# pyannote/pyannote-audio

Measured on NVIDIA H100. Metric: audio-hours/sec (RTF) community-1 diarization, 16kHz mono, 1/2/4/8 H100, higher is better.
Workload: dtype f16 tensor-core trunk (f32 accumulate) + split-f16x3 tensor-core segmentation (f32-level accuracy) + f64 clustering

## Files before the change

### pyannote_audio_b200/csrc/api.cu

```cuda
#include "../../include/b200diar.h"
#include "audio.cuh"
#include "cluster.cuh"
#include "common.cuh"
#include "emb.cuh"
#include "post.cuh"
#include "seg.cuh"
#include "ssl.cuh"
#include <algorithm>
#include <climits>
#include <cmath>
#include <cstdlib>

using namespace b200;

constexpr int kXvecLayers = 5;
constexpr int kXvecMinSamples = 4771;
constexpr int kXvecStatsLd = 3008;
struct XvecWeights {
  bool loaded = false;
  SincNetWeights sinc;
  int taps[kXvecLayers] = {5, 3, 3, 1, 1}, dil[kXvecLayers] = {1, 2, 3, 1, 1};
  int cin_pad[kXvecLayers] = {64, 512, 512, 512, 512}, cout_pad[kXvecLayers] = {512, 512, 512, 512, 1536};
  __half* w_hi[kXvecLayers] = {};
  __half* w_lo[kXvecLayers] = {};
// ... 365 lines not shown
        }
    if ((rc = upload_split(ctx, whh_wg, &S.w_hh_hi[l], &S.w_hh_lo[l]))) return rc;
  }
  const int lin_in[2] = {256, 128};
  for (int i = 0; i < 2; ++i) {
    B200_CHECK(w->linear_weight[i] && w->linear_bias[i], B200_ERR_INVALID, "linear.%d missing", i);
    std::vector<float> lw(w->linear_weight[i], w->linear_weight[i] + 128 * lin_in[i]), lb(w->linear_bias[i], w->linear_bias[i] + 128);
    if ((rc = upload_split(ctx, lw, &S.lin_w_hi[i], &S.lin_w_lo[i]))) return rc;
    if ((rc = upload(ctx, lw, &S.lin_w[i]))) return rc;
    if ((rc = upload(ctx, lb, &S.lin_b[i]))) return rc;
  }
  B200_CHECK(w->classifier_weight && w->classifier_bias, B200_ERR_INVALID, "classifier missing");
  std::vector<float> cw(w->classifier_weight, w->classifier_weight + (size_t)num_classes * 128),
      cb(w->classifier_bias, w->classifier_bias + num_classes);
  if ((rc = upload(ctx, cw, &S.cls_w))) return rc;
  if ((rc = upload(ctx, cb, &S.cls_b))) return rc;
  return B200_OK;
}

}

extern "C" {

const char* b200_last_error(void) { return b200::last_error(); }
int b200_version(void) { return 100; }

int b200_ctx_create(b200_ctx** out, int device) {
  B200_CHECK(out != nullptr, B200_ERR_INVALID, "ctx pointer is NULL");
  int ndev = 0;
  B200_CUDA_OK(cudaGetDeviceCount(&ndev));
  B200_CHECK(device >= 0 && device < ndev, B200_ERR_INVALID, "device %d not available (%d devices)", device, ndev);
  cudaDeviceProp prop;
  B200_CUDA_OK(cudaGetDeviceProperties(&prop, device));
  B200_CHECK(prop.major == 9 && prop.minor == 0, B200_ERR_STATE,
             "device %d is sm_%d%d; this library is built for sm_90a (H100) only", device, prop.major, prop.minor);
  b200_ctx* c = new b200_ctx();
  c->device = device;
  c->num_sms = prop.multiProcessorCount;
  if (const char* e = std::getenv("B200_CONV_IMPL")) c->conv_impl = std::atoi(e);
  if (const char* e = std::getenv("B200_EMB_MAX_BATCH")) c->emb_max_batch = std::atoi(e) > 0 ? std::atoi(e) : c->emb_max_batch;
  if (const char* e = std::getenv("B200_SEG_MAX_BATCH")) c->seg_max_batch = std::atoi(e) > 0 ? std::atoi(e) : c->seg_max_batch;
  *out = c;
  return B200_OK;
}

int b200_ctx_destroy(b200_ctx* ctx) {
  if (!ctx) return B200_OK;
  DeviceGuard g(ctx->device);
  cudaDeviceSynchronize();
  for (void* p : ctx->owned_seg) cudaFree(p);
  for (void* p : ctx->owned_emb) cudaFree(p);
  for (void* p : ctx->owned_xvec) cudaFree(p);
  for (void* p : ctx->owned_ssl) cudaFree(p);
  for (auto& t : ctx->resample_tables) cudaFree(t.dev);
  if (ctx->ws) cudaFree(ctx->ws);
  if (ctx->d_off) cudaFree(ctx->d_off);
  if (ctx->d_valid) cudaFree(ctx->d_valid);
  if (ctx->d_frame0) cudaFree(ctx->d_frame0);
  if (ctx->d_runs) cudaFree(ctx->d_runs);
  delete ctx;
  return B200_OK;
}

int b200_ctx_set_option(b200_ctx* ctx, const char* key, int64_t value) {
  B200_CHECK(ctx && key, B200_ERR_INVALID, "NULL ctx/key");
  std::string k(key);
  if (k == "conv_impl") ctx->conv_impl = (int)value;
  else if (k == "seg_max_batch") ctx->seg_max_batch = (int)value;
  else if (k == "emb_max_batch") ctx->emb_max_batch = (int)value;
  else if (k == "ssl_max_batch") ctx->ssl_max_batch = (int)value;
  else if (k == "profile") ctx->profile = (int)value;
  else if (k == "seg_gemm_impl") ctx->seg_gemm_impl = (int)value;
  else if (k == "seg_conv_impl") ctx->seg_conv_impl = (int)value;
  else if (k == "seg_rec_impl") ctx->seg_rec_impl = (int)value;
  else if (k == "fbank_share") ctx->fbank_share = (int)value;
  else if (k == "linkage_grid_min") {
    B200_CHECK(value >= 2 && value <= kLinkGridMinDefault, B200_ERR_INVALID, "option '%s' value %lld out of range",
               key, (long long)value);
    ctx->linkage_grid_min = (int)value;
  }
  else B200_CHECK(false, B200_ERR_INVALID, "unknown option '%s'", key);
  B200_CHECK(ctx->seg_max_batch >= 1 && ctx->emb_max_batch >= 1 && ctx->ssl_max_batch >= 1 && ctx->conv_impl >= 0 && ctx->conv_impl <= 2 &&
                 ctx->seg_gemm_impl >= 0 && ctx->seg_gemm_impl <= 1 && ctx->seg_conv_impl >= 0 && ctx->seg_conv_impl <= 2 &&
                 ctx->seg_rec_impl >= 0 && ctx->seg_rec_impl <= 1,
             B200_ERR_INVALID, "option '%s' value %lld out of range", key, (long long)value);
  return B200_OK;
}

int64_t b200_ctx_launch_count(const b200_ctx* ctx) { return ctx ? ctx->launches : 0; }

int b200_ctx_timer(b200_ctx* ctx, const char* name, double* total_ms, int64_t* units) {
  B200_CHECK(ctx && name && total_ms && units, B200_ERR_INVALID, "bad arguments");
  DeviceGuard g(ctx->device);
  std::string k(name);
  std::vector<std::pair<cudaEvent_t, cudaEvent_t>>* v = nullptr;
  int64_t* u = nullptr;
  if (k == "trunk") { v = &ctx->trunk_events; u = &ctx->trunk_segments; }
  else if (k == "seg") { v = &ctx->seg_events; u = &ctx->seg_chunks; }
  else B200_CHECK(false, B200_ERR_INVALID, "unknown timer '%s'", name);
  B200_CUDA_OK(cudaDeviceSynchronize());
  double ms = 0.0;
  for (auto& pr : *v) {
    float t = 0.f;
    B200_CUDA_OK(cudaEventElapsedTime(&t, pr.first, pr.second));
    ms += t;
    ctx->event_pool.push_back(pr.first);
    ctx->event_pool.push_back(pr.second);
  }
  v->clear();
  *total_ms = ms;
  *units = *u;
  *u = 0;
  return B200_OK;
}

static int64_t gcd64(int64_t a, int64_t b) { while (b) { const int64_t t = a % b; a = b; b = t; } return a; }

int64_t b200_audio_num_frames(int64_t frames_in, int32_t sr_in, int32_t sr_out) {
  if (frames_in <= 0 || sr_in <= 0 || sr_out <= 0) return 0;
  if (sr_in == sr_out) return frames_in;
  const int64_t g = gcd64(sr_in, sr_out), orig = sr_in / g, nw = sr_out / g;
  return (nw * frames_in + orig - 1) / orig;
}

int b200_audio_ingest(b200_ctx* ctx, const void* pcm, int32_t format, int32_t channels, int64_t frames_in,
                      int32_t sr_in, int32_t sr_out, int32_t channel, float* out, int64_t out_capacity, void* stream) {
  B200_CHECK(ctx && pcm && out && channels >= 1 && frames_in >= 0 && sr_in > 0 && sr_out > 0, B200_ERR_INVALID,
             "bad arguments");
  B200_CHECK(format == B200_PCM_S16_INTERLEAVED || format == B200_PCM_F32_PLANAR, B200_ERR_INVALID,
             "unknown PCM format %d", (int)format);
  B200_CHECK(channel < channels, B200_ERR_INVALID, "channel %d of a %d-channel file", (int)channel, (int)channels);
  const int64_t frames_out = b200_audio_num_frames(frames_in, sr_in, sr_out);
  B200_CHECK(frames_out <= out_capacity, B200_ERR_INVALID, "output holds %lld samples, %lld needed",
             (long long)out_capacity, (long long)frames_out);
  if (frames_out == 0) return B200_OK;
  DeviceGuard g(ctx->device);
  const int64_t gg = gcd64(sr_in, sr_out);
  const int orig = (int)(sr_in / gg), nw = (int)(sr_out / gg);
  const b200_ctx::ResampleTable* tab = nullptr;
  for (auto& t : ctx->resample_tables)
    if (t.orig == orig && t.nw == nw) tab = &t;
  if (!tab) {
    b200_ctx::ResampleTable t{orig, nw, 0, nullptr};
    std::vector<float> host;
    if (orig == nw) { host.assign(1, 1.0f); t.width = 0; }
    else resample_table(orig, nw, &t.width, &host);
    B200_CUDA_OK(cudaMalloc((void**)&t.dev, host.size() * sizeof(float)));
    B200_CUDA_OK(cudaMemcpy(t.dev, host.data(), host.size() * sizeof(float), cudaMemcpyHostToDevice));
    ctx->resample_tables.push_back(t);
    tab = &ctx->resample_tables.back();
  }
  ctx->launches += 1;
  return audio_ingest(pcm, format, channels, frames_in, channel, tab->dev, tab->orig, tab->nw, tab->width, out,
                      frames_out, (cudaStream_t)stream);
}

int b200_seg_load_head(b200_ctx* ctx, const b200_seg_weights* w, int32_t num_classes, int32_t activation) {
  B200_CHECK(ctx && w, B200_ERR_INVALID, "NULL ctx/weights");
  B200_CHECK(num_classes >= 1 && num_classes <= kSegMaxClasses, B200_ERR_INVALID,
             "a classifier of %d classes is unsupported (1 .. %d)", (int)num_classes, kSegMaxClasses);
  B200_CHECK(activation == B200_SEG_LOGSOFTMAX || activation == B200_SEG_SIGMOID, B200_ERR_INVALID,
             "unknown classifier activation %d (B200_SEG_LOGSOFTMAX = 0, B200_SEG_SIGMOID = 1)", (int)activation);
  DeviceGuard g(ctx->device);
  SegWeights& S = ctx->seg;
  B200_CHECK(w->lstm_layers >= 1 && w->lstm_layers <= 4, B200_ERR_INVALID, "lstm_layers=%d unsupported",
             (int)w->lstm_layers);
  S.loaded = false;
// ... 1031 lines not shown
```

### pyannote_audio_b200/csrc/seg.cuh

```cuda
#pragma once
#include "common.cuh"

namespace b200 {

constexpr int kSegMinWindow = 1261;
constexpr int kSegTileP = 64;
struct SegGeom {
  int W, sinc_len, pool0, conv1_len, pool1, conv2_len, pool2;
  int tiles0, tiles1, tiles2;
};
inline SegGeom seg_geom(int W) {
  SegGeom g;
  g.W = W;
  g.sinc_len = 1 + (W - kSincK) / kSincStride;
  g.pool0 = g.sinc_len / 3;
  g.conv1_len = g.pool0 - 4;
  g.pool1 = g.conv1_len / 3;
  g.conv2_len = g.pool1 - 4;
  g.pool2 = g.conv2_len / 3;
  g.tiles0 = (g.pool0 + kSegTileP - 1) / kSegTileP;
  g.tiles1 = (g.pool1 + kSegTileP - 1) / kSegTileP;
  g.tiles2 = (g.pool2 + kSegTileP - 1) / kSegTileP;
  return g;
}

struct SincNetWeights {
  float wav_w = 1.f, wav_b = 0.f;
  __half* sinc_wg_hi = nullptr;
  __half* sinc_wg_lo = nullptr;
  float* sinc_f = nullptr;
  float* in_gamma[3] = {nullptr, nullptr, nullptr};
  float* in_beta[3] = {nullptr, nullptr, nullptr};
  float* conv_w[2] = {nullptr, nullptr};
  float* conv_b[2] = {nullptr, nullptr};
  __half* conv_wg_hi[2] = {nullptr, nullptr};
  __half* conv_wg_lo[2] = {nullptr, nullptr};
};

constexpr int kSegLogSoftmax = 0;
constexpr int kSegSigmoid = 1;
constexpr int kSegMaxClasses = 32;

struct SegWeights {
  bool loaded = false;
  int lstm_layers = 4;
  int num_classes = kClasses;
  int activation = kSegLogSoftmax;
  SincNetWeights sinc;
  float* w_ih[8] = {};
  float* b_g[8] = {};
  int k_in[8] = {};
  float* w_hh[8] = {};
  __half* w_hh_hi[8] = {};
  __half* w_hh_lo[8] = {};
  __half* w_ih_hi[8] = {};
  __half* w_ih_lo[8] = {};
  __half* lin_w_hi[2] = {nullptr, nullptr};
  __half* lin_w_lo[2] = {nullptr, nullptr};
  float* lin_w[2] = {nullptr, nullptr};
  float* lin_b[2] = {nullptr, nullptr};
  float* cls_w = nullptr;
  float* cls_b = nullptr;
};

int sgemm_nt(const float* A, int lda, const float* Bw, int ldb, float* C, int ldc, const float* bias, int M, int N,
             int K, int act, cudaStream_t stream);

struct GemmTaps {
  int taps = 1, dil = 0;
  const float* scale = nullptr;
  const float* shift = nullptr;
};
int gemm_tc_split(const __half* A_hi, const __half* A_lo, int lda, const __half* B_hi, const __half* B_lo, int ldb,
                  float* C, int ldc, __half* C_hi, __half* C_lo, int ldc_h, const float* bias, int M, int N, int K,
                  int act, int num_sms, cudaStream_t stream, float* const* C_peers = nullptr, int n_peers = 0,
                  const GemmTaps& taps = GemmTaps());
int split_f16(const float* x, __half* hi, __half* lo, size_t n, cudaStream_t st);
int lstm_rec_wg(const float* Gx, const __half* Wh, const __half* Wl, __half* Yh, __half* Yl, int NB, int T,
                cudaStream_t stream);

int sinc_wg_forward(const SegGeom& g, const float* wav, const long long* chunk_off, const int* chunk_valid,
                    const float2* affine, const __half* Wh, const __half* Wl, int NB, float* P0, double2* part,
                    int impl, cudaStream_t stream);
int conv5_wg_forward(const SegGeom& g, int layer, const float* Pin, const float2* affine, const __half* Wh,
                     const __half* Wl, const float* bias, int NB, float* Pout, double2* part, int impl,
                     cudaStream_t stream);

size_t sincnet_workspace_bytes(const SegGeom& g, int NB);
int sincnet_launches(const SegGeom& g);
int sincnet_forward(const SincNetWeights& W, const SegGeom& g, const float* wav, const long long* chunk_off,
                    const int* chunk_valid, int NB, void* ws, float* x0, int conv_impl, cudaStream_t stream);

struct SegHeadOut {
  unsigned char* cls = nullptr;
  float* logp = nullptr;
  float* scores = nullptr;
  float* max_scores = nullptr;
};
size_t lstm_workspace_bytes(int NB, int T, int k0);
int lstm_head_forward(const SegWeights& W, const float* x0, int NB, int T, void* ws, const SegHeadOut& out,
                      int num_sms, int gemm_impl, int rec_impl, cudaStream_t stream);

}
```

### pyannote_audio_b200/csrc/seg_lstm.cu

```cuda
#include "common.cuh"
#include "seg.cuh"
#include <cooperative_groups.h>
#include <array>
#include <utility>

namespace cg = cooperative_groups;

namespace b200 {

__device__ __forceinline__ float sigmoidf_(float x) { return 1.f / (1.f + expf(-x)); }

template <int RB>
__global__ void __cluster_dims__(2, 1, 1) __launch_bounds__(256, 1)
lstm_rec_kernel(const float* __restrict__ Gx , const float* __restrict__ Whh ,
                float* __restrict__ Y , __half* __restrict__ Yh, __half* __restrict__ Yl,
                int NB, int T, int ntiles) {
  constexpr int NBT = 8 * RB;
  extern __shared__ float sm[];
  float* Ws = sm;
  float* hb = sm + 128 * 256;
  cg::cluster_group cluster = cg::this_cluster();
  const int rank = (int)cluster.block_rank();
  const int cid = blockIdx.x >> 1;
  const int dir = cid / ntiles;
// ... 142 lines not shown
  for (int k = 1; k < K; ++k) mx = fmaxf(mx, v[k]);
  float se = 0.f;
#pragma unroll
  for (int k = 0; k < K; ++k) se += expf(v[k] - mx);
  const float lse = logf(se);
  int best = 0;
  float bv = 0.f;
#pragma unroll
  for (int k = 0; k < K; ++k) {
    const float lp = (v[k] - mx) - lse;
    if (logp) logp[(size_t)row * K + k] = lp;
    if (k == 0 || lp > bv) { bv = lp; best = k; }
  }
  cls[row] = (unsigned char)best;
}

typedef void (*ClassifierFn)(const float*, const float*, const float*, unsigned char*, float*, float*, float*, int);
template <int ACT, int... I>
static std::array<ClassifierFn, sizeof...(I)> classifier_table(std::integer_sequence<int, I...>) {
  return {{&classifier_kernel<I + 1, ACT>...}};
}
static const auto kLogSoftmaxHeads = classifier_table<kSegLogSoftmax>(std::make_integer_sequence<int, kSegMaxClasses>());
static const auto kSigmoidHeads = classifier_table<kSegSigmoid>(std::make_integer_sequence<int, kSegMaxClasses>());

struct LstmWs {
  float *Gx, *Ya, *Yb, *Z1, *Z2;
  __half *Xh, *Xl, *Yah, *Yal, *Ybh, *Ybl, *Z1h, *Z1l;
};
static size_t carve_lstm(int NB, int T, int k0, void* base, LstmWs* w) {
  Workspace ws(base, 256);
  LstmWs t;
  const size_t M = (size_t)NB * T;
  t.Gx = (float*)ws.take(M * 1024 * sizeof(float));
  t.Ya = (float*)ws.take(M * 256 * sizeof(float));
  t.Yb = (float*)ws.take(M * 256 * sizeof(float));
  t.Z1 = (float*)ws.take(M * 128 * sizeof(float));
  t.Z2 = (float*)ws.take(M * 128 * sizeof(float));
  t.Xh = (__half*)ws.take(M * k0 * sizeof(__half));
  t.Xl = (__half*)ws.take(M * k0 * sizeof(__half));
  t.Yah = (__half*)ws.take(M * 256 * sizeof(__half));
  t.Yal = (__half*)ws.take(M * 256 * sizeof(__half));
  t.Ybh = (__half*)ws.take(M * 256 * sizeof(__half));
  t.Ybl = (__half*)ws.take(M * 256 * sizeof(__half));
  t.Z1h = (__half*)ws.take(M * 128 * sizeof(__half));
  t.Z1l = (__half*)ws.take(M * 128 * sizeof(__half));
  if (w) *w = t;
  return ws.bytes();
}
size_t lstm_workspace_bytes(int NB, int T, int k0) { return carve_lstm(NB, T, k0, nullptr, nullptr); }

template <int RB>
static int launch_rec(const float* Gx, const float* Whh, float* Y, __half* Yh, __half* Yl, int NB, int T,
                      cudaStream_t stream) {
  constexpr int NBT = 8 * RB;
  const int ntiles = ceil_div(NB, NBT);
  const size_t smem = (128 * 256 + 2 * 128 * NBT) * sizeof(float);
  B200_CUDA_OK(cudaFuncSetAttribute(lstm_rec_kernel<RB>, cudaFuncAttributeMaxDynamicSharedMemorySize, (int)smem));
  lstm_rec_kernel<RB><<<2 * 2 * ntiles, 256, smem, stream>>>(Gx, Whh, Y, Yh, Yl, NB, T, ntiles);
  B200_CUDA_OK(cudaGetLastError());
  return B200_OK;
}

int lstm_head_forward(const SegWeights& W, const float* x0, int NB, int T, void* ws, const SegHeadOut& out,
                      int num_sms, int gemm_impl, int rec_impl, cudaStream_t stream) {
  LstmWs w;
  carve_lstm(NB, T, W.k_in[0], ws, &w);
  const int M = NB * T;
  const int clusters = num_sms / 2;
  const bool tc = gemm_impl != 0;
  int rc;
  const float* in = x0;
  const __half *in_h = w.Xh, *in_l = w.Xl;
  if (tc && (rc = split_f16(x0, w.Xh, w.Xl, (size_t)M * W.k_in[0], stream))) return rc;
  float* outs[2] = {w.Ya, w.Yb};
  __half* outs_h[2] = {w.Yah, w.Ybh};
  __half* outs_l[2] = {w.Yal, w.Ybl};
  for (int l = 0; l < W.lstm_layers; ++l) {
    if (tc)
      rc = gemm_tc_split(in_h, in_l, W.k_in[l], W.w_ih_hi[l], W.w_ih_lo[l], W.k_in[l], w.Gx, 1024, nullptr, nullptr, 0,
                         W.b_g[l], M, 1024, W.k_in[l], 0, num_sms, stream);
    else
      rc = sgemm_nt(in, W.k_in[l], W.w_ih[l], W.k_in[l], w.Gx, 1024, W.b_g[l], M, 1024, W.k_in[l], 0, stream);
    if (rc) return rc;
    if (tc && rec_impl == 1) {
      if ((rc = lstm_rec_wg(w.Gx, W.w_hh_hi[l], W.w_hh_lo[l], outs_h[l & 1], outs_l[l & 1], NB, T, stream))) return rc;
      in_h = outs_h[l & 1]; in_l = outs_l[l & 1];
      continue;
    }
    float* y = tc ? nullptr : outs[l & 1];
    __half* yh = tc ? outs_h[l & 1] : nullptr;
    __half* yl = tc ? outs_l[l & 1] : nullptr;
    if (2 * ceil_div(NB, 64) >= clusters) rc = launch_rec<8>(w.Gx, W.w_hh[l], y, yh, yl, NB, T, stream);
    else if (2 * ceil_div(NB, 32) >= clusters) rc = launch_rec<4>(w.Gx, W.w_hh[l], y, yh, yl, NB, T, stream);
    else rc = launch_rec<2>(w.Gx, W.w_hh[l], y, yh, yl, NB, T, stream);
    if (rc) return rc;
    in = y; in_h = yh; in_l = yl;
  }
  if (tc) {
    rc = gemm_tc_split(in_h, in_l, 256, W.lin_w_hi[0], W.lin_w_lo[0], 256, nullptr, 0, w.Z1h, w.Z1l, 128, W.lin_b[0], M,
                       128, 256, 1, num_sms, stream);
    if (rc) return rc;
    rc = gemm_tc_split(w.Z1h, w.Z1l, 128, W.lin_w_hi[1], W.lin_w_lo[1], 128, w.Z2, 128, nullptr, nullptr, 0,
                       W.lin_b[1], M, 128, 128, 1, num_sms, stream);
    if (rc) return rc;
  } else {
    rc = sgemm_nt(in, 256, W.lin_w[0], 256, w.Z1, 128, W.lin_b[0], M, 128, 256, 1, stream);
    if (rc) return rc;
    rc = sgemm_nt(w.Z1, 128, W.lin_w[1], 128, w.Z2, 128, W.lin_b[1], M, 128, 128, 1, stream);
    if (rc) return rc;
  }
  const ClassifierFn head = (W.activation == kSegSigmoid ? kSigmoidHeads : kLogSoftmaxHeads)[W.num_classes - 1];
  head<<<ceil_div(M, 8), 256, 0, stream>>>(w.Z2, W.cls_w, W.cls_b, out.cls, out.logp, out.scores, out.max_scores, M);
  B200_CUDA_OK(cudaGetLastError());
  return B200_OK;
}

}
```

### pyannote_audio_b200/csrc/seg_lstm_wg.cu

```cuda
#include "common.cuh"
#include "seg.cuh"
#include "tc_common.cuh"

namespace b200 {

constexpr int kRecThreads = 128;
constexpr int kRecSeqs = 64;
constexpr uint32_t kRecWBox = 256u * 128u;
constexpr uint32_t kRecXOff = 1024u + 4u * kRecWBox;

__device__ __forceinline__ float rec_sigmoid(float x) { return 1.f / (1.f + expf(-x)); }

__device__ __forceinline__ uint32_t pack_h2(float a, float b) {
  __half2 h = __floats2half2_rn(a, b);
  return *reinterpret_cast<uint32_t*>(&h);
}

__global__ void __cluster_dims__(2, 1, 1) __launch_bounds__(kRecThreads, 1)
lstm_rec_wg_kernel(const __grid_constant__ CUtensorMap tmWh, const __grid_constant__ CUtensorMap tmWl,
                   const float* __restrict__ Gx , __half* __restrict__ Yh, __half* __restrict__ Yl,
                   int NB, int T, int ntiles) {
  extern __shared__ uint8_t smem_raw[];
  const uint32_t raw = smem_u32(smem_raw);
  const uint32_t base = (raw + 1023u) & ~1023u;
// ... 33 lines not shown

  float acc[128];
  for (int step = 0; step < T; ++step) {
    const int t = dir ? (T - 1 - step) : step;
#pragma unroll
    for (int i = 0; i < 2; ++i) {
      const bool ok = rows[i] < NB;
      const float4* gp = reinterpret_cast<const float4*>(Gx + ((size_t)(ok ? rows[i] : 0) * T + t) * 1024 + gcol);
#pragma unroll
      for (int jj = 0; jj < 8; ++jj) {
        const float4 u0 = ok ? __ldg(gp + 8 * jj) : make_float4(0.f, 0.f, 0.f, 0.f);
        const float4 u1 = ok ? __ldg(gp + 8 * jj + 1) : make_float4(0.f, 0.f, 0.f, 0.f);
        const float v[8] = {u0.x, u0.y, u0.z, u0.w, u1.x, u1.y, u1.z, u1.w};
#pragma unroll
        for (int g = 0; g < 4; ++g)
#pragma unroll
          for (int e = 0; e < 2; ++e) acc[4 * (4 * jj + g) + 2 * i + e] = v[4 * e + g];
      }
      if (step + 1 < T && ok) {
        const int tn = dir ? t - 1 : t + 1;
        const char* np = reinterpret_cast<const char*>(Gx + ((size_t)rows[i] * T + tn) * 1024 + gcol);
#pragma unroll
        for (int jj = 0; jj < 8; ++jj) asm volatile("prefetch.global.L2 [%0];" ::"l"(np + 128 * jj));
      }
    }
    wg_fence();
#pragma unroll
    for (int ks = 0; ks < 8; ++ks) {
      const int s = ks & 3;
      const uint32_t* xb = xbuf + ((step & 1) * 2 + (ks >> 2)) * 32 * kRecThreads;
      uint32_t ah[4], al[4];
#pragma unroll
      for (int r = 0; r < 4; ++r) {
        const int i = r & 1, jj = 2 * s + (r >> 1);
        ah[r] = xb[(i * 8 + jj) * kRecThreads + tid];
        al[r] = xb[(16 + i * 8 + jj) * kRecThreads + tid];
      }
      const uint32_t wb = w_smem + (uint32_t)(ks >> 2) * kRecWBox + (uint32_t)(ks & 3) * 32u;
      const uint64_t wh = wg_desc(wb, 128), wl = wg_desc(wb + 2 * kRecWBox, 128);
      WgmmaRS<256>::mma(acc, al, wh);
      WgmmaRS<256>::mma(acc, ah, wl);
      WgmmaRS<256>::mma(acc, ah, wh);
    }
    wg_commit();
    wg_wait<0>();
    const uint32_t hoff = (uint32_t)((((step + 1) & 1) * 2 + (int)rank) * 32 * kRecThreads + tid);
    uint32_t* own = xbuf + hoff;
    const uint32_t px = peer_x + hoff * 4u;
#pragma unroll
    for (int i = 0; i < 2; ++i) {
#pragma unroll
      for (int jj = 0; jj < 8; ++jj) {
        float hn[2];
#pragma unroll
        for (int e = 0; e < 2; ++e) {
          const float ig = rec_sigmoid(acc[4 * (4 * jj + 0) + 2 * i + e]);
          const float fg = rec_sigmoid(acc[4 * (4 * jj + 1) + 2 * i + e]);
          const float gg = tanhf(acc[4 * (4 * jj + 2) + 2 * i + e]);
          const float og = rec_sigmoid(acc[4 * (4 * jj + 3) + 2 * i + e]);
          c[i][jj][e] = fmaf(fg, c[i][jj][e], ig * gg);
          hn[e] = og * tanhf(c[i][jj][e]);
        }
        const __half h0 = __float2half_rn(hn[0]), h1 = __float2half_rn(hn[1]);
        const __half2 hi2 = __halves2half2(h0, h1);
        const uint32_t vh = *reinterpret_cast<const uint32_t*>(&hi2);
        const uint32_t vl = pack_h2(hn[0] - __half2float(h0), hn[1] - __half2float(h1));
        own[(i * 8 + jj) * kRecThreads] = vh;
        own[(16 + i * 8 + jj) * kRecThreads] = vl;
        asm volatile("st.shared::cluster.u32 [%0], %1;" ::"r"(px + (uint32_t)((i * 8 + jj) * kRecThreads) * 4u),
                     "r"(vh) : "memory");
        asm volatile("st.shared::cluster.u32 [%0], %1;" ::"r"(px + (uint32_t)((16 + i * 8 + jj) * kRecThreads) * 4u),
                     "r"(vl) : "memory");
        if (rows[i] < NB) {
          const size_t o = ((size_t)rows[i] * T + t) * 256 + dir * 128 + rank * 64 + 8 * jj + 2 * q;
          *reinterpret_cast<uint32_t*>(Yh + o) = vh;
          *reinterpret_cast<uint32_t*>(Yl + o) = vl;
        }
      }
    }
    asm volatile("barrier.cluster.arrive.release.aligned;\n\tbarrier.cluster.wait.acquire.aligned;" ::: "memory");
  }
}

int lstm_rec_wg(const float* Gx, const __half* Wh, const __half* Wl, __half* Yh, __half* Yl, int NB, int T,
                cudaStream_t stream) {
  CUtensorMap tm[2];
  const cuuint64_t dims[3] = {128, 256, 4};
  const cuuint64_t strides[2] = {128 * 2, 256 * 128 * 2};
  const cuuint32_t box[3] = {64, 256, 1};
  int rc;
  for (int h = 0; h < 2; ++h)
    if ((rc = encode_f16_map(&tm[h], 3, h ? Wl : Wh, dims, strides, box, nullptr, CU_TENSOR_MAP_SWIZZLE_128B,
                             "lstm W_hh")))
      return rc;
  const size_t smem = 1024 + kRecXOff + 4u * 32u * kRecThreads * 4u;
  B200_CUDA_OK(cudaFuncSetAttribute(lstm_rec_wg_kernel, cudaFuncAttributeMaxDynamicSharedMemorySize, (int)smem));
  const int ntiles = ceil_div(NB, kRecSeqs);
  lstm_rec_wg_kernel<<<2 * 2 * ntiles, kRecThreads, smem, stream>>>(tm[0], tm[1], Gx, Yh, Yl, NB, T, ntiles);
  B200_CUDA_OK(cudaGetLastError());
  return B200_OK;
}

}
```

### pyannote_audio_b200/csrc/tc_common.cuh

```cuda
#pragma once
#include "common.cuh"
#include <cuda.h>

namespace b200 {

__device__ __forceinline__ uint32_t smem_u32(const void* p) {
  return static_cast<uint32_t>(__cvta_generic_to_shared(p));
}
__device__ __forceinline__ void mbar_init(uint32_t bar, uint32_t count) {
  asm volatile("mbarrier.init.shared::cta.b64 [%0], %1;" ::"r"(bar), "r"(count));
}
__device__ __forceinline__ void mbar_expect_tx(uint32_t bar, uint32_t bytes) {
  asm volatile("mbarrier.arrive.expect_tx.shared::cta.b64 _, [%0], %1;" ::"r"(bar), "r"(bytes) : "memory");
}
__device__ __forceinline__ void mbar_arrive(uint32_t bar) {
  asm volatile("mbarrier.arrive.shared::cta.b64 _, [%0];" ::"r"(bar) : "memory");
}
__device__ __forceinline__ void mbar_arrive_n(uint32_t bar, uint32_t count) {
  asm volatile("mbarrier.arrive.shared::cta.b64 _, [%0], %1;" ::"r"(bar), "r"(count) : "memory");
}
__device__ __forceinline__ void mbar_wait(uint32_t bar, uint32_t parity) {
  asm volatile(
      "{\n\t"
      ".reg .pred p;\n\t"
// ... 52 lines not shown
}
__device__ __forceinline__ void named_bar_sync(int id) { asm volatile("bar.sync %0, 128;" ::"r"(id) : "memory"); }
__device__ __forceinline__ void wg_fence() { asm volatile("wgmma.fence.sync.aligned;" ::: "memory"); }
__device__ __forceinline__ void wg_commit() { asm volatile("wgmma.commit_group.sync.aligned;" ::: "memory"); }
template <int N>
__device__ __forceinline__ void wg_wait() { asm volatile("wgmma.wait_group.sync.aligned %0;" ::"n"(N) : "memory"); }

template <int N>
struct Wgmma;
template <>
struct Wgmma<32> {
  __device__ __forceinline__ static void mma(float* d, uint64_t a, uint64_t b) {
    asm volatile(
        "wgmma.mma_async.sync.aligned.m64n32k16.f32.f16.f16 "
        "{%0, %1, %2, %3, %4, %5, %6, %7, %8, %9, %10, %11, %12, %13, %14, %15}, %16, %17, 1, 1, 1, 0, 0;"
        : "+f"(d[0]), "+f"(d[1]), "+f"(d[2]), "+f"(d[3]), "+f"(d[4]), "+f"(d[5]), "+f"(d[6]), "+f"(d[7]), "+f"(d[8]), "+f"(d[9]), "+f"(d[10]), "+f"(d[11]), "+f"(d[12]), "+f"(d[13]), "+f"(d[14]), "+f"(d[15])
        : "l"(a), "l"(b));
  }
};
template <>
struct Wgmma<64> {
  __device__ __forceinline__ static void mma(float* d, uint64_t a, uint64_t b) {
    asm volatile(
        "wgmma.mma_async.sync.aligned.m64n64k16.f32.f16.f16 "
        "{%0, %1, %2, %3, %4, %5, %6, %7, %8, %9, %10, %11, %12, %13, %14, %15, %16, %17, %18, %19, %20, %21, %22, %23, %24, %25, %26, %27, %28, %29, %30, %31}, %32, %33, 1, 1, 1, 0, 0;"
        : "+f"(d[0]), "+f"(d[1]), "+f"(d[2]), "+f"(d[3]), "+f"(d[4]), "+f"(d[5]), "+f"(d[6]), "+f"(d[7]), "+f"(d[8]), "+f"(d[9]), "+f"(d[10]), "+f"(d[11]), "+f"(d[12]), "+f"(d[13]), "+f"(d[14]), "+f"(d[15]), "+f"(d[16]), "+f"(d[17]), "+f"(d[18]), "+f"(d[19]), "+f"(d[20]), "+f"(d[21]), "+f"(d[22]), "+f"(d[23]), "+f"(d[24]), "+f"(d[25]), "+f"(d[26]), "+f"(d[27]), "+f"(d[28]), "+f"(d[29]), "+f"(d[30]), "+f"(d[31])
        : "l"(a), "l"(b));
  }
};
template <>
struct Wgmma<128> {
  __device__ __forceinline__ static void mma(float* d, uint64_t a, uint64_t b) {
    asm volatile(
        "wgmma.mma_async.sync.aligned.m64n128k16.f32.f16.f16 "
        "{%0, %1, %2, %3, %4, %5, %6, %7, %8, %9, %10, %11, %12, %13, %14, %15, %16, %17, %18, %19, %20, %21, %22, %23, %24, %25, %26, %27, %28, %29, %30, %31, %32, %33, %34, %35, %36, %37, %38, %39, %40, %41, %42, %43, %44, %45, %46, %47, %48, %49, %50, %51, %52, %53, %54, %55, %56, %57, %58, %59, %60, %61, %62, %63}, %64, %65, 1, 1, 1, 0, 0;"
        : "+f"(d[0]), "+f"(d[1]), "+f"(d[2]), "+f"(d[3]), "+f"(d[4]), "+f"(d[5]), "+f"(d[6]), "+f"(d[7]), "+f"(d[8]), "+f"(d[9]), "+f"(d[10]), "+f"(d[11]), "+f"(d[12]), "+f"(d[13]), "+f"(d[14]), "+f"(d[15]), "+f"(d[16]), "+f"(d[17]), "+f"(d[18]), "+f"(d[19]), "+f"(d[20]), "+f"(d[21]), "+f"(d[22]), "+f"(d[23]), "+f"(d[24]), "+f"(d[25]), "+f"(d[26]), "+f"(d[27]), "+f"(d[28]), "+f"(d[29]), "+f"(d[30]), "+f"(d[31]), "+f"(d[32]), "+f"(d[33]), "+f"(d[34]), "+f"(d[35]), "+f"(d[36]), "+f"(d[37]), "+f"(d[38]), "+f"(d[39]), "+f"(d[40]), "+f"(d[41]), "+f"(d[42]), "+f"(d[43]), "+f"(d[44]), "+f"(d[45]), "+f"(d[46]), "+f"(d[47]), "+f"(d[48]), "+f"(d[49]), "+f"(d[50]), "+f"(d[51]), "+f"(d[52]), "+f"(d[53]), "+f"(d[54]), "+f"(d[55]), "+f"(d[56]), "+f"(d[57]), "+f"(d[58]), "+f"(d[59]), "+f"(d[60]), "+f"(d[61]), "+f"(d[62]), "+f"(d[63])
        : "l"(a), "l"(b));
  }
};
template <>
struct Wgmma<256> {
  __device__ __forceinline__ static void mma(float* d, uint64_t a, uint64_t b) {
    asm volatile(
        "wgmma.mma_async.sync.aligned.m64n256k16.f32.f16.f16 "
        "{%0, %1, %2, %3, %4, %5, %6, %7, %8, %9, %10, %11, %12, %13, %14, %15, %16, %17, %18, %19, %20, %21, %22, %23, %24, %25, %26, %27, %28, %29, %30, %31, %32, %33, %34, %35, %36, %37, %38, %39, %40, %41, %42, %43, %44, %45, %46, %47, %48, %49, %50, %51, %52, %53, %54, %55, %56, %57, %58, %59, %60, %61, %62, %63, %64, %65, %66, %67, %68, %69, %70, %71, %72, %73, %74, %75, %76, %77, %78, %79, %80, %81, %82, %83, %84, %85, %86, %87, %88, %89, %90, %91, %92, %93, %94, %95, %96, %97, %98, %99, %100, %101, %102, %103, %104, %105, %106, %107, %108, %109, %110, %111, %112, %113, %114, %115, %116, %117, %118, %119, %120, %121, %122, %123, %124, %125, %126, %127}, %128, %129, 1, 1, 1, 0, 0;"
        : "+f"(d[0]), "+f"(d[1]), "+f"(d[2]), "+f"(d[3]), "+f"(d[4]), "+f"(d[5]), "+f"(d[6]), "+f"(d[7]), "+f"(d[8]), "+f"(d[9]), "+f"(d[10]), "+f"(d[11]), "+f"(d[12]), "+f"(d[13]), "+f"(d[14]), "+f"(d[15]), "+f"(d[16]), "+f"(d[17]), "+f"(d[18]), "+f"(d[19]), "+f"(d[20]), "+f"(d[21]), "+f"(d[22]), "+f"(d[23]), "+f"(d[24]), "+f"(d[25]), "+f"(d[26]), "+f"(d[27]), "+f"(d[28]), "+f"(d[29]), "+f"(d[30]), "+f"(d[31]), "+f"(d[32]), "+f"(d[33]), "+f"(d[34]), "+f"(d[35]), "+f"(d[36]), "+f"(d[37]), "+f"(d[38]), "+f"(d[39]), "+f"(d[40]), "+f"(d[41]), "+f"(d[42]), "+f"(d[43]), "+f"(d[44]), "+f"(d[45]), "+f"(d[46]), "+f"(d[47]), "+f"(d[48]), "+f"(d[49]), "+f"(d[50]), "+f"(d[51]), "+f"(d[52]), "+f"(d[53]), "+f"(d[54]), "+f"(d[55]), "+f"(d[56]), "+f"(d[57]), "+f"(d[58]), "+f"(d[59]), "+f"(d[60]), "+f"(d[61]), "+f"(d[62]), "+f"(d[63]), "+f"(d[64]), "+f"(d[65]), "+f"(d[66]), "+f"(d[67]), "+f"(d[68]), "+f"(d[69]), "+f"(d[70]), "+f"(d[71]), "+f"(d[72]), "+f"(d[73]), "+f"(d[74]), "+f"(d[75]), "+f"(d[76]), "+f"(d[77]), "+f"(d[78]), "+f"(d[79]), "+f"(d[80]), "+f"(d[81]), "+f"(d[82]), "+f"(d[83]), "+f"(d[84]), "+f"(d[85]), "+f"(d[86]), "+f"(d[87]), "+f"(d[88]), "+f"(d[89]), "+f"(d[90]), "+f"(d[91]), "+f"(d[92]), "+f"(d[93]), "+f"(d[94]), "+f"(d[95]), "+f"(d[96]), "+f"(d[97]), "+f"(d[98]), "+f"(d[99]), "+f"(d[100]), "+f"(d[101]), "+f"(d[102]), "+f"(d[103]), "+f"(d[104]), "+f"(d[105]), "+f"(d[106]), "+f"(d[107]), "+f"(d[108]), "+f"(d[109]), "+f"(d[110]), "+f"(d[111]), "+f"(d[112]), "+f"(d[113]), "+f"(d[114]), "+f"(d[115]), "+f"(d[116]), "+f"(d[117]), "+f"(d[118]), "+f"(d[119]), "+f"(d[120]), "+f"(d[121]), "+f"(d[122]), "+f"(d[123]), "+f"(d[124]), "+f"(d[125]), "+f"(d[126]), "+f"(d[127])
        : "l"(a), "l"(b));
  }
};

template <int N>
struct WgmmaRS;
template <>
struct WgmmaRS<32> {
  __device__ __forceinline__ static void mma(float* d, const uint32_t* a, uint64_t b) {
    asm volatile(
        "wgmma.mma_async.sync.aligned.m64n32k16.f32.f16.f16 "
        "{%0, %1, %2, %3, %4, %5, %6, %7, %8, %9, %10, %11, %12, %13, %14, %15}, {%16, %17, %18, %19}, %20, 1, 1, 1, 0;"
        : "+f"(d[0]), "+f"(d[1]), "+f"(d[2]), "+f"(d[3]), "+f"(d[4]), "+f"(d[5]), "+f"(d[6]), "+f"(d[7]), "+f"(d[8]), "+f"(d[9]), "+f"(d[10]), "+f"(d[11]), "+f"(d[12]), "+f"(d[13]), "+f"(d[14]), "+f"(d[15])
        : "r"(a[0]), "r"(a[1]), "r"(a[2]), "r"(a[3]), "l"(b));
  }
};
template <>
struct WgmmaRS<64> {
  __device__ __forceinline__ static void mma(float* d, const uint32_t* a, uint64_t b) {
    asm volatile(
        "wgmma.mma_async.sync.aligned.m64n64k16.f32.f16.f16 "
        "{%0, %1, %2, %3, %4, %5, %6, %7, %8, %9, %10, %11, %12, %13, %14, %15, %16, %17, %18, %19, %20, %21, %22, %23, %24, %25, %26, %27, %28, %29, %30, %31}, {%32, %33, %34, %35}, %36, 1, 1, 1, 0;"
        : "+f"(d[0]), "+f"(d[1]), "+f"(d[2]), "+f"(d[3]), "+f"(d[4]), "+f"(d[5]), "+f"(d[6]), "+f"(d[7]), "+f"(d[8]), "+f"(d[9]), "+f"(d[10]), "+f"(d[11]), "+f"(d[12]), "+f"(d[13]), "+f"(d[14]), "+f"(d[15]), "+f"(d[16]), "+f"(d[17]), "+f"(d[18]), "+f"(d[19]), "+f"(d[20]), "+f"(d[21]), "+f"(d[22]), "+f"(d[23]), "+f"(d[24]), "+f"(d[25]), "+f"(d[26]), "+f"(d[27]), "+f"(d[28]), "+f"(d[29]), "+f"(d[30]), "+f"(d[31])
        : "r"(a[0]), "r"(a[1]), "r"(a[2]), "r"(a[3]), "l"(b));
  }
};
template <>
struct WgmmaRS<80> {
  __device__ __forceinline__ static void mma(float* d, const uint32_t* a, uint64_t b) {
    asm volatile(
        "wgmma.mma_async.sync.aligned.m64n80k16.f32.f16.f16 "
        "{%0, %1, %2, %3, %4, %5, %6, %7, %8, %9, %10, %11, %12, %13, %14, %15, %16, %17, %18, %19, %20, %21, %22, %23, %24, %25, %26, %27, %28, %29, %30, %31, %32, %33, %34, %35, %36, %37, %38, %39}, {%40, %41, %42, %43}, %44, 1, 1, 1, 0;"
        : "+f"(d[0]), "+f"(d[1]), "+f"(d[2]), "+f"(d[3]), "+f"(d[4]), "+f"(d[5]), "+f"(d[6]), "+f"(d[7]), "+f"(d[8]), "+f"(d[9]), "+f"(d[10]), "+f"(d[11]), "+f"(d[12]), "+f"(d[13]), "+f"(d[14]), "+f"(d[15]), "+f"(d[16]), "+f"(d[17]), "+f"(d[18]), "+f"(d[19]), "+f"(d[20]), "+f"(d[21]), "+f"(d[22]), "+f"(d[23]), "+f"(d[24]), "+f"(d[25]), "+f"(d[26]), "+f"(d[27]), "+f"(d[28]), "+f"(d[29]), "+f"(d[30]), "+f"(d[31]), "+f"(d[32]), "+f"(d[33]), "+f"(d[34]), "+f"(d[35]), "+f"(d[36]), "+f"(d[37]), "+f"(d[38]), "+f"(d[39])
        : "r"(a[0]), "r"(a[1]), "r"(a[2]), "r"(a[3]), "l"(b));
  }
};
template <>
struct WgmmaRS<256> {
  __device__ __forceinline__ static void mma(float* d, const uint32_t* a, uint64_t b) {
    asm volatile(
        "wgmma.mma_async.sync.aligned.m64n256k16.f32.f16.f16 "
        "{%0, %1, %2, %3, %4, %5, %6, %7, %8, %9, %10, %11, %12, %13, %14, %15, %16, %17, %18, %19, %20, %21, %22, %23, %24, %25, %26, %27, %28, %29, %30, %31, %32, %33, %34, %35, %36, %37, %38, %39, %40, %41, %42, %43, %44, %45, %46, %47, %48, %49, %50, %51, %52, %53, %54, %55, %56, %57, %58, %59, %60, %61, %62, %63, %64, %65, %66, %67, %68, %69, %70, %71, %72, %73, %74, %75, %76, %77, %78, %79, %80, %81, %82, %83, %84, %85, %86, %87, %88, %89, %90, %91, %92, %93, %94, %95, %96, %97, %98, %99, %100, %101, %102, %103, %104, %105, %106, %107, %108, %109, %110, %111, %112, %113, %114, %115, %116, %117, %118, %119, %120, %121, %122, %123, %124, %125, %126, %127}, {%128, %129, %130, %131}, %132, 1, 1, 1, 0;"
        : "+f"(d[0]), "+f"(d[1]), "+f"(d[2]), "+f"(d[3]), "+f"(d[4]), "+f"(d[5]), "+f"(d[6]), "+f"(d[7]), "+f"(d[8]), "+f"(d[9]), "+f"(d[10]), "+f"(d[11]), "+f"(d[12]), "+f"(d[13]), "+f"(d[14]), "+f"(d[15]), "+f"(d[16]), "+f"(d[17]), "+f"(d[18]), "+f"(d[19]), "+f"(d[20]), "+f"(d[21]), "+f"(d[22]), "+f"(d[23]), "+f"(d[24]), "+f"(d[25]), "+f"(d[26]), "+f"(d[27]), "+f"(d[28]), "+f"(d[29]), "+f"(d[30]), "+f"(d[31]), "+f"(d[32]), "+f"(d[33]), "+f"(d[34]), "+f"(d[35]), "+f"(d[36]), "+f"(d[37]), "+f"(d[38]), "+f"(d[39]), "+f"(d[40]), "+f"(d[41]), "+f"(d[42]), "+f"(d[43]), "+f"(d[44]), "+f"(d[45]), "+f"(d[46]), "+f"(d[47]), "+f"(d[48]), "+f"(d[49]), "+f"(d[50]), "+f"(d[51]), "+f"(d[52]), "+f"(d[53]), "+f"(d[54]), "+f"(d[55]), "+f"(d[56]), "+f"(d[57]), "+f"(d[58]), "+f"(d[59]), "+f"(d[60]), "+f"(d[61]), "+f"(d[62]), "+f"(d[63]), "+f"(d[64]), "+f"(d[65]), "+f"(d[66]), "+f"(d[67]), "+f"(d[68]), "+f"(d[69]), "+f"(d[70]), "+f"(d[71]), "+f"(d[72]), "+f"(d[73]), "+f"(d[74]), "+f"(d[75]), "+f"(d[76]), "+f"(d[77]), "+f"(d[78]), "+f"(d[79]), "+f"(d[80]), "+f"(d[81]), "+f"(d[82]), "+f"(d[83]), "+f"(d[84]), "+f"(d[85]), "+f"(d[86]), "+f"(d[87]), "+f"(d[88]), "+f"(d[89]), "+f"(d[90]), "+f"(d[91]), "+f"(d[92]), "+f"(d[93]), "+f"(d[94]), "+f"(d[95]), "+f"(d[96]), "+f"(d[97]), "+f"(d[98]), "+f"(d[99]), "+f"(d[100]), "+f"(d[101]), "+f"(d[102]), "+f"(d[103]), "+f"(d[104]), "+f"(d[105]), "+f"(d[106]), "+f"(d[107]), "+f"(d[108]), "+f"(d[109]), "+f"(d[110]), "+f"(d[111]), "+f"(d[112]), "+f"(d[113]), "+f"(d[114]), "+f"(d[115]), "+f"(d[116]), "+f"(d[117]), "+f"(d[118]), "+f"(d[119]), "+f"(d[120]), "+f"(d[121]), "+f"(d[122]), "+f"(d[123]), "+f"(d[124]), "+f"(d[125]), "+f"(d[126]), "+f"(d[127])
        : "r"(a[0]), "r"(a[1]), "r"(a[2]), "r"(a[3]), "l"(b));
  }
};

int encode_f16_map(CUtensorMap* tm, int rank, const void* ptr, const cuuint64_t* dims, const cuuint64_t* strides,
                   const cuuint32_t* box, const cuuint32_t* estr, CUtensorMapSwizzle swizzle, const char* what);

}
```

Baseline: 1.908.

## Add two-warpgroup pipelined LSTM recurrence kernel as default rec impl

Adds a new LSTM recurrence kernel that splits the 256 gate columns across two warpgroups, each issuing m64n128 split-f16 wgmma, and prefetches the next step's Gx input while the tensor-core work runs. The cluster barrier is split into arrive and wait halves so the wait for the peer's h exchange overlaps the Yh/Yl global stores. With rec_impl=1 as the default, the new kernel replaces the old one, which stays reachable as impl 2. In exchange the kernel uses more threads and registers and adds a little code complexity.

```diff
diff --git a/pyannote_audio_b200/csrc/api.cu b/pyannote_audio_b200/csrc/api.cu
--- a/pyannote_audio_b200/csrc/api.cu
+++ b/pyannote_audio_b200/csrc/api.cu
@@ -471,7 +471,7 @@
   else B200_CHECK(false, B200_ERR_INVALID, "unknown option '%s'", key);
   B200_CHECK(ctx->seg_max_batch >= 1 && ctx->emb_max_batch >= 1 && ctx->ssl_max_batch >= 1 && ctx->conv_impl >= 0 && ctx->conv_impl <= 2 &&
                  ctx->seg_gemm_impl >= 0 && ctx->seg_gemm_impl <= 1 && ctx->seg_conv_impl >= 0 && ctx->seg_conv_impl <= 2 &&
-                 ctx->seg_rec_impl >= 0 && ctx->seg_rec_impl <= 1,
+                 ctx->seg_rec_impl >= 0 && ctx->seg_rec_impl <= 2,
              B200_ERR_INVALID, "option '%s' value %lld out of range", key, (long long)value);
   return B200_OK;
 }
diff --git a/pyannote_audio_b200/csrc/seg.cuh b/pyannote_audio_b200/csrc/seg.cuh
--- a/pyannote_audio_b200/csrc/seg.cuh
+++ b/pyannote_audio_b200/csrc/seg.cuh
@@ -76,7 +76,7 @@
                   int act, int num_sms, cudaStream_t stream, float* const* C_peers = nullptr, int n_peers = 0,
                   const GemmTaps& taps = GemmTaps());
 int split_f16(const float* x, __half* hi, __half* lo, size_t n, cudaStream_t st);
-int lstm_rec_wg(const float* Gx, const __half* Wh, const __half* Wl, __half* Yh, __half* Yl, int NB, int T,
+int lstm_rec_wg(const float* Gx, const __half* Wh, const __half* Wl, __half* Yh, __half* Yl, int NB, int T, int impl,
                 cudaStream_t stream);
 
 int sinc_wg_forward(const SegGeom& g, const float* wav, const long long* chunk_off, const int* chunk_valid,
diff --git a/pyannote_audio_b200/csrc/seg_lstm.cu b/pyannote_audio_b200/csrc/seg_lstm.cu
--- a/pyannote_audio_b200/csrc/seg_lstm.cu
+++ b/pyannote_audio_b200/csrc/seg_lstm.cu
@@ -248,8 +248,9 @@
     else
       rc = sgemm_nt(in, W.k_in[l], W.w_ih[l], W.k_in[l], w.Gx, 1024, W.b_g[l], M, 1024, W.k_in[l], 0, stream);
     if (rc) return rc;
-    if (tc && rec_impl == 1) {
-      if ((rc = lstm_rec_wg(w.Gx, W.w_hh_hi[l], W.w_hh_lo[l], outs_h[l & 1], outs_l[l & 1], NB, T, stream))) return rc;
+    if (tc && rec_impl != 0) {
+      if ((rc = lstm_rec_wg(w.Gx, W.w_hh_hi[l], W.w_hh_lo[l], outs_h[l & 1], outs_l[l & 1], NB, T, rec_impl, stream)))
+        return rc;
       in_h = outs_h[l & 1]; in_l = outs_l[l & 1];
       continue;
     }
diff --git a/pyannote_audio_b200/csrc/seg_lstm_wg.cu b/pyannote_audio_b200/csrc/seg_lstm_wg.cu
--- a/pyannote_audio_b200/csrc/seg_lstm_wg.cu
+++ b/pyannote_audio_b200/csrc/seg_lstm_wg.cu
@@ -139,7 +139,163 @@
   }
 }
 
-int lstm_rec_wg(const float* Gx, const __half* Wh, const __half* Wl, __half* Yh, __half* Yl, int NB, int T,
+struct RecPipePlan {
+  static constexpr int kWarpgroups = 2;
+  static constexpr int kThreads = 128 * kWarpgroups;
+  static constexpr int kCols = 256 / kWarpgroups;
+  static constexpr uint32_t kBar = 0;
+  static constexpr uint32_t kW = 1024;
+  static constexpr uint32_t kWgColBytes = (uint32_t)kCols * 128u;
+  static constexpr uint32_t kX = kW + 4u * kRecWBox;
+  static constexpr uint32_t kXBytes = 2u * 2u * 32u * 128u * 4u;
+  static constexpr size_t kSmem = 1024 + kX + kXBytes;
+  static_assert(kX == kRecXOff, "same h buffer offset as the reference kernel");
+  static_assert(kW % 1024 == 0 && kRecWBox % 1024 == 0 && kWgColBytes % 1024 == 0,
+                "128-byte swizzle atoms (8 rows of 128 B) must start 1024-byte aligned");
+  static_assert(kCols * kWarpgroups == 256 && kCols == 128, "each warpgroup runs m64n128");
+  static_assert(kSmem <= 227u * 1024u, "one CTA per SM");
+};
+
+__global__ void __cluster_dims__(2, 1, 1) __launch_bounds__(RecPipePlan::kThreads, 1)
+lstm_rec_pipe_kernel(const __grid_constant__ CUtensorMap tmWh, const __grid_constant__ CUtensorMap tmWl,
+                     const float* __restrict__ Gx , __half* __restrict__ Yh, __half* __restrict__ Yl,
+                     int NB, int T, int ntiles) {
+  using P = RecPipePlan;
+  extern __shared__ uint8_t smem_raw[];
+  const uint32_t raw = smem_u32(smem_raw);
+  const uint32_t base = (raw + 1023u) & ~1023u;
+  const uint32_t bar = base + P::kBar, w_smem = base + P::kW;
+  uint32_t* xbuf = reinterpret_cast<uint32_t*>(smem_raw + (base - raw) + P::kX);
+  uint32_t rank;
+  asm volatile("mov.u32 %0, %%cluster_ctarank;" : "=r"(rank));
+  const int cid = blockIdx.x >> 1;
+  const int dir = cid / ntiles, tile = cid - dir * ntiles;
+  const int tid = threadIdx.x, wg = tid >> 7, t128 = tid & 127, warp = t128 >> 5, lane = tid & 31, q = lane & 3;
+  uint32_t peer_x;
+  asm volatile("mapa.shared::cluster.u32 %0, %1, %2;" : "=r"(peer_x) : "r"(base + P::kX), "r"(rank ^ 1u));
+
+  if (tid == 0) {
+    mbar_init(bar, 1);
+    asm volatile("fence.mbarrier_init.release.cluster;" ::: "memory");
+    mbar_expect_tx(bar, 4u * kRecWBox);
+    const int slice = dir * 2 + (int)rank;
+    tma_load_3d(&tmWh, bar, w_smem, 0, 0, slice);
+    tma_load_3d(&tmWh, bar, w_smem + kRecWBox, 64, 0, slice);
+    tma_load_3d(&tmWl, bar, w_smem + 2 * kRecWBox, 0, 0, slice);
+    tma_load_3d(&tmWl, bar, w_smem + 3 * kRecWBox, 64, 0, slice);
+  }
+  for (int i = tid; i < 2 * 32 * 128; i += P::kThreads) xbuf[i] = 0u;
+  asm volatile("barrier.cluster.arrive.release.aligned;\n\tbarrier.cluster.wait.acquire.aligned;" ::: "memory");
+  mbar_wait(bar, 0);
+
+  int rows[2];
+  rows[0] = tile * kRecSeqs + 16 * warp + (lane >> 2);
+  rows[1] = rows[0] + 8;
+  const bool ok[2] = {rows[0] < NB, rows[1] < NB};
+  float c[2][4][2];
+#pragma unroll
+  for (int i = 0; i < 2; ++i)
+#pragma unroll
+    for (int j = 0; j < 4; ++j) c[i][j][0] = c[i][j][1] = 0.f;
+  const int gcol = dir * 512 + ((int)rank * 64 + 32 * wg + 2 * q) * 4;
+
+  float gx[64];
+  auto load_gx = [&](int t) {
+#pragma unroll
+    for (int i = 0; i < 2; ++i) {
+      const float4* gp = reinterpret_cast<const float4*>(Gx + ((size_t)(ok[i] ? rows[i] : 0) * T + t) * 1024 + gcol);
+#pragma unroll
+      for (int j = 0; j < 4; ++j) {
+        const float4 u0 = ok[i] ? __ldg(gp + 8 * j) : make_float4(0.f, 0.f, 0.f, 0.f);
+        const float4 u1 = ok[i] ? __ldg(gp + 8 * j + 1) : make_float4(0.f, 0.f, 0.f, 0.f);
+        const float v[8] = {u0.x, u0.y, u0.z, u0.w, u1.x, u1.y, u1.z, u1.w};
+#pragma unroll
+        for (int g = 0; g < 4; ++g)
+#pragma unroll
+          for (int e = 0; e < 2; ++e) gx[4 * (4 * j + g) + 2 * i + e] = v[4 * e + g];
+      }
+    }
+  };
+  load_gx(dir ? T - 1 : 0);
+  asm volatile("barrier.cluster.arrive.release.aligned;" ::: "memory");
+
+  const uint32_t w_wg = w_smem + (uint32_t)wg * P::kWgColBytes;
+  float acc[64];
+  for (int step = 0; step < T; ++step) {
+    const int t = dir ? (T - 1 - step) : step;
+#pragma unroll
+    for (int r = 0; r < 64; ++r) acc[r] = gx[r];
+    asm volatile("barrier.cluster.wait.acquire.aligned;" ::: "memory");
+    wg_fence();
+#pragma unroll
+    for (int ks = 0; ks < 8; ++ks) {
+      const int s = ks & 3;
+      const uint32_t* xb = xbuf + ((step & 1) * 2 + (ks >> 2)) * 32 * 128;
+      uint32_t ah[4], al[4];
+#pragma unroll
+      for (int r = 0; r < 4; ++r) {
+        const int i = r & 1, jj = 2 * s + (r >> 1);
+        ah[r] = xb[(i * 8 + jj) * 128 + t128];
+        al[r] = xb[(16 + i * 8 + jj) * 128 + t128];
+      }
+      const uint32_t wb = w_wg + (uint32_t)(ks >> 2) * kRecWBox + (uint32_t)(ks & 3) * 32u;
+      const uint64_t wh = wg_desc(wb, 128), wl = wg_desc(wb + 2 * kRecWBox, 128);
+      WgmmaRS<P::kCols>::mma(acc, al, wh);
+      WgmmaRS<P::kCols>::mma(acc, ah, wl);
+      WgmmaRS<P::kCols>::mma(acc, ah, wh);
+    }
+    wg_commit();
+    if (step + 1 < T) load_gx(dir ? t - 1 : t + 1);
+    wg_wait<0>();
+    const uint32_t hoff = (uint32_t)((((step + 1) & 1) * 2 + (int)rank) * 32 * 128 + t128);
+    uint32_t* own = xbuf + hoff;
+    const uint32_t px = peer_x + hoff * 4u;
+    uint32_t yv[2][4][2];
+#pragma unroll
+    for (int i = 0; i < 2; ++i) {
+#pragma unroll
+      for (int j = 0; j < 4; ++j) {
+        const int jj = 4 * wg + j;
+        float hn[2];
+#pragma unroll
+        for (int e = 0; e < 2; ++e) {
+          const float ig = rec_sigmoid(acc[4 * (4 * j + 0) + 2 * i + e]);
+          const float fg = rec_sigmoid(acc[4 * (4 * j + 1) + 2 * i + e]);
+          const float gg = tanhf(acc[4 * (4 * j + 2) + 2 * i + e]);
+          const float og = rec_sigmoid(acc[4 * (4 * j + 3) + 2 * i + e]);
+          c[i][j][e] = fmaf(fg, c[i][j][e], ig * gg);
+          hn[e] = og * tanhf(c[i][j][e]);
+        }
+        const __half h0 = __float2half_rn(hn[0]), h1 = __float2half_rn(hn[1]);
+        const __half2 hi2 = __halves2half2(h0, h1);
+        const uint32_t vh = *reinterpret_cast<const uint32_t*>(&hi2);
+        const uint32_t vl = pack_h2(hn[0] - __half2float(h0), hn[1] - __half2float(h1));
+        own[(i * 8 + jj) * 128] = vh;
+        own[(16 + i * 8 + jj) * 128] = vl;
+        asm volatile("st.shared::cluster.u32 [%0], %1;" ::"r"(px + (uint32_t)((i * 8 + jj) * 128) * 4u), "r"(vh)
+                     : "memory");
+        asm volatile("st.shared::cluster.u32 [%0], %1;" ::"r"(px + (uint32_t)((16 + i * 8 + jj) * 128) * 4u), "r"(vl)
+                     : "memory");
+        yv[i][j][0] = vh;
+        yv[i][j][1] = vl;
+      }
+    }
+    asm volatile("barrier.cluster.arrive.release.aligned;" ::: "memory");
+#pragma unroll
+    for (int i = 0; i < 2; ++i) {
+      if (!ok[i]) continue;
+      const size_t o = ((size_t)rows[i] * T + t) * 256 + dir * 128 + rank * 64 + 32 * wg + 2 * q;
+#pragma unroll
+      for (int j = 0; j < 4; ++j) {
+        *reinterpret_cast<uint32_t*>(Yh + o + 8 * j) = yv[i][j][0];
+        *reinterpret_cast<uint32_t*>(Yl + o + 8 * j) = yv[i][j][1];
+      }
+    }
+  }
+  asm volatile("barrier.cluster.wait.acquire.aligned;" ::: "memory");
+}
+
+int lstm_rec_wg(const float* Gx, const __half* Wh, const __half* Wl, __half* Yh, __half* Yl, int NB, int T, int impl,
                 cudaStream_t stream) {
   CUtensorMap tm[2];
   const cuuint64_t dims[3] = {128, 256, 4};
@@ -150,10 +306,17 @@
     if ((rc = encode_f16_map(&tm[h], 3, h ? Wl : Wh, dims, strides, box, nullptr, CU_TENSOR_MAP_SWIZZLE_128B,
                              "lstm W_hh")))
       return rc;
-  const size_t smem = 1024 + kRecXOff + 4u * 32u * kRecThreads * 4u;
-  B200_CUDA_OK(cudaFuncSetAttribute(lstm_rec_wg_kernel, cudaFuncAttributeMaxDynamicSharedMemorySize, (int)smem));
   const int ntiles = ceil_div(NB, kRecSeqs);
-  lstm_rec_wg_kernel<<<2 * 2 * ntiles, kRecThreads, smem, stream>>>(tm[0], tm[1], Gx, Yh, Yl, NB, T, ntiles);
+  if (impl == 1) {
+    const size_t smem = RecPipePlan::kSmem;
+    B200_CUDA_OK(cudaFuncSetAttribute(lstm_rec_pipe_kernel, cudaFuncAttributeMaxDynamicSharedMemorySize, (int)smem));
+    lstm_rec_pipe_kernel<<<2 * 2 * ntiles, RecPipePlan::kThreads, smem, stream>>>(tm[0], tm[1], Gx, Yh, Yl, NB, T,
+                                                                                  ntiles);
+  } else {
+    const size_t smem = 1024 + kRecXOff + 4u * 32u * kRecThreads * 4u;
+    B200_CUDA_OK(cudaFuncSetAttribute(lstm_rec_wg_kernel, cudaFuncAttributeMaxDynamicSharedMemorySize, (int)smem));
+    lstm_rec_wg_kernel<<<2 * 2 * ntiles, kRecThreads, smem, stream>>>(tm[0], tm[1], Gx, Yh, Yl, NB, T, ntiles);
+  }
   B200_CUDA_OK(cudaGetLastError());
   return B200_OK;
 }
diff --git a/pyannote_audio_b200/csrc/tc_common.cuh b/pyannote_audio_b200/csrc/tc_common.cuh
--- a/pyannote_audio_b200/csrc/tc_common.cuh
+++ b/pyannote_audio_b200/csrc/tc_common.cuh
@@ -158,6 +158,16 @@
   }
 };
 template <>
+struct WgmmaRS<128> {
+  __device__ __forceinline__ static void mma(float* d, const uint32_t* a, uint64_t b) {
+    asm volatile(
+        "wgmma.mma_async.sync.aligned.m64n128k16.f32.f16.f16 "
+        "{%0, %1, %2, %3, %4, %5, %6, %7, %8, %9, %10, %11, %12, %13, %14, %15, %16, %17, %18, %19, %20, %21, %22, %23, %24, %25, %26, %27, %28, %29, %30, %31, %32, %33, %34, %35, %36, %37, %38, %39, %40, %41, %42, %43, %44, %45, %46, %47, %48, %49, %50, %51, %52, %53, %54, %55, %56, %57, %58, %59, %60, %61, %62, %63}, {%64, %65, %66, %67}, %68, 1, 1, 1, 0;"
+        : "+f"(d[0]), "+f"(d[1]), "+f"(d[2]), "+f"(d[3]), "+f"(d[4]), "+f"(d[5]), "+f"(d[6]), "+f"(d[7]), "+f"(d[8]), "+f"(d[9]), "+f"(d[10]), "+f"(d[11]), "+f"(d[12]), "+f"(d[13]), "+f"(d[14]), "+f"(d[15]), "+f"(d[16]), "+f"(d[17]), "+f"(d[18]), "+f"(d[19]), "+f"(d[20]), "+f"(d[21]), "+f"(d[22]), "+f"(d[23]), "+f"(d[24]), "+f"(d[25]), "+f"(d[26]), "+f"(d[27]), "+f"(d[28]), "+f"(d[29]), "+f"(d[30]), "+f"(d[31]), "+f"(d[32]), "+f"(d[33]), "+f"(d[34]), "+f"(d[35]), "+f"(d[36]), "+f"(d[37]), "+f"(d[38]), "+f"(d[39]), "+f"(d[40]), "+f"(d[41]), "+f"(d[42]), "+f"(d[43]), "+f"(d[44]), "+f"(d[45]), "+f"(d[46]), "+f"(d[47]), "+f"(d[48]), "+f"(d[49]), "+f"(d[50]), "+f"(d[51]), "+f"(d[52]), "+f"(d[53]), "+f"(d[54]), "+f"(d[55]), "+f"(d[56]), "+f"(d[57]), "+f"(d[58]), "+f"(d[59]), "+f"(d[60]), "+f"(d[61]), "+f"(d[62]), "+f"(d[63])
+        : "r"(a[0]), "r"(a[1]), "r"(a[2]), "r"(a[3]), "l"(b));
+  }
+};
+template <>
 struct WgmmaRS<256> {
   __device__ __forceinline__ static void mma(float* d, const uint32_t* a, uint64_t b) {
     asm volatile(
```

After: 1.965 (median of 6 runs). 1.03x the previous value.
